# ChaissonLab/LRA

Measured on AMD Instinct MI355X. Metric: aligned Gbp/s, 30 kb ONT vs GRCh38 (MapRead_lowacc end to end incl. SAM text), per job, higher is better.
Workload: dtype int32

## Files before the change

### lra_amd/csrc/indel_refine.hip

```cpp
#include "common.h"
#include "scan.h"
#include <algorithm>
#include <stdlib.h>

int lra_aog_launch_device(lra_ctx* ctx, int n, const char* d_qseq, const char* d_tseq, const uint64_t* d_q_off,
                          const int32_t* d_q_len, const uint64_t* d_t_off, const int32_t* d_t_len, const int32_t* d_k,
                          int m, int mm, int indel, int32_t* d_score, int32_t* d_nblocks, int32_t* d_blocks,
                          const uint64_t* d_block_off, int32_t* d_status);

namespace {

constexpr int BAD = -999999999;
constexpr int NEG = -2000000000;
enum { C_DIAG = 0, C_LEFT = 1, C_DOWN = 2, C_BOUND = 3, C_DELCLOSE = 4, C_INSCLOSE = 5, C_DONE = 6 };

__device__ __forceinline__ void wave_sync() {
  __builtin_amdgcn_fence(__ATOMIC_RELEASE, "workgroup");
  __builtin_amdgcn_wave_barrier();
  __builtin_amdgcn_fence(__ATOMIC_ACQUIRE, "workgroup");
}

__device__ __forceinline__ void wave_sync_lds() {
  __builtin_amdgcn_fence(__ATOMIC_RELEASE, "wavefront");
  __builtin_amdgcn_wave_barrier();
// ... 307 lines not shown
  int status = B.s_status[s];
  const long tLen = (long)B.s_rows[s];
  Row* rows = B.rows + B.s_row_off[s];
  unsigned long long cells = 0;
  int width = 0;
  if (!status && tLen > 0) {
    int run = 0x7fffffff;
    for (long base = ((tLen - 1) / 64) * 64; base >= 0; base -= 64) {
      const long r = base + lane;
      const int own = (r < tLen) ? rows[r].S : 0x7fffffff;
      int v = own;
      for (int d = 1; d < 64; d <<= 1) { int o = __shfl_down(v, d); if (lane + d < 64) v = min(v, o); }
      v = min(v, run);
      if (r < tLen && v != own) rows[r].S = v;
      run = __shfl(v, 0);
    }
    const int a = B.s_aln[s];
    const unsigned char* tb = (const unsigned char*)B.tseq + B.t_off[a] + B.s_tStart[s];
    int runE = -0x7fffffff;
    for (long base = 0; base < tLen; base += 64) {
      const long r = base + lane;
      Row w; w.S = 0; w.E = -0x7fffffff; w.C = 0; w.T = 0;
      if (r < tLen) w = rows[r];
      int e = w.E;
      for (int d = 1; d < 64; d <<= 1) { int o = __shfl_up(e, d); if (lane >= d) e = max(e, o); }
      e = max(e, runE);
      runE = __shfl(e, 63);
      int len = (r < tLen) ? e - w.S + 1 : 0;
      if (r < tLen) {
        if (len < 1 || w.S < 0) status |= 1;
        else if (len > MAXW) status |= 4;
        width = max(width, len);
      }
      const unsigned long long l = (unsigned long long)max(len, 0);
      unsigned long long inc = l;
      for (int d = 1; d < 64; d <<= 1) { unsigned long long o = __shfl_up(inc, d); if (lane >= d) inc += o; }
      if (r < tLen) { w.E = e; w.C = (unsigned int)(cells + inc - l); w.T = tb[r]; rows[r] = w; }
      cells += __shfl(inc, 63);
    }
    for (int o = 32; o > 0; o >>= 1) { status |= __shfl_xor(status, o); width = max(width, __shfl_xor(width, o)); }
  }
  if (lane == 0) {
    B.s_cells[s] = status ? 0 : cells;
    B.s_status[s] = status;
    B.s_width[s] = status ? 0 : width;
    B.s_tmpcap[s] = status ? 0 : (uint64_t)(tLen + ((long)B.s_qEnd[s] - B.s_qStart[s]) + 2);
  }
}

constexpr int FILL_BINS = 128;
template <bool EMIT>
__global__ void ir_classify(uint64_t n_seg, const int32_t* __restrict__ s_kind, const int32_t* __restrict__ s_status, const int32_t* __restrict__ s_width,
                            const uint64_t* __restrict__ s_rows, int* bins, uint32_t* list) {
  const uint64_t s = (uint64_t)blockIdx.x * blockDim.x + threadIdx.x;
  const int lane = threadIdx.x & 63;
  int bin = -1;
  if (s < n_seg && s_kind[s] == 0 && s_status[s] == 0) {
    const int w = s_width[s];
    const uint32_t r = (uint32_t)min((unsigned long long)s_rows[s], 0x7fffffffULL);
    bin = (w <= 16 ? 0 : w <= 32 ? 1 : w <= 64 ? 2 : 3) * 32 + (r ? __clz(r) : 31);
  }
  const unsigned long long below = (lane == 0) ? 0ULL : (~0ULL >> (64 - lane));
  unsigned long long todo = __ballot(bin >= 0);
  while (todo) {
    const int leader = __ffsll((long long)todo) - 1;
    const int b = __shfl(bin, leader);
    const unsigned long long m = __ballot(bin == b);
    int base = 0;
    if (lane == leader) base = atomicAdd(&bins[b], __popcll(m));
    base = __shfl(base, leader);
    if (EMIT && bin == b) list[base + __popcll(m & below)] = (uint32_t)s;
    todo &= ~m;
  }
}

struct FillArgs {
  uint64_t n_seg;
  const int32_t* s_aln; const uint64_t* s_rows; const uint64_t* s_row_off; const uint64_t* s_cell_off;
  const Row* rows;
  const char* qseq; const uint64_t* q_off; const int32_t* q_len;
  int match, mismatch, g;
  unsigned char* path;
  const uint32_t* list; int* cursor;
};

__device__ __forceinline__ bool is_bound(long row, int c, int len) { return c == len - 1 || (row > 0 && c == 0); }

__device__ __forceinline__ int shr1(int x, int fill) { return __builtin_amdgcn_update_dpp(fill, x, 0x138, 0xf, 0xf, false); }
template <int G>
__device__ __forceinline__ int scan_max(int w) {
  w = max(w, __builtin_amdgcn_update_dpp(NEG, w, 0x111, 0xf, 0xf, false));
  w = max(w, __builtin_amdgcn_update_dpp(NEG, w, 0x112, 0xf, 0xf, false));
  w = max(w, __builtin_amdgcn_update_dpp(NEG, w, 0x114, 0xf, 0xf, false));
  w = max(w, __builtin_amdgcn_update_dpp(NEG, w, 0x118, 0xf, 0xf, false));
  if (G >= 32) w = max(w, __builtin_amdgcn_update_dpp(NEG, w, 0x142, 0xa, 0xf, false));
  if (G >= 64) w = max(w, __builtin_amdgcn_update_dpp(NEG, w, 0x143, 0xc, 0xf, false));
  return w;
}

template <int G>
__global__ void __launch_bounds__(64) ir_fill(FillArgs F) {
  constexpr int GP = 64 / G;
  constexpr int CLS = (G == 16) ? 0 : (G == 32) ? 1 : 2;
  const int lane = threadIdx.x;
  const int c = lane % G, gbase = lane - c;
  const int g = F.g, go = 2 * F.g + 1;
  const long listEnd = F.cursor[4 + CLS];
  const uint32_t* list = F.list;
  long ti = -1, tLen = 0;
  const Row* rows = nullptr; const unsigned char* qb = nullptr; unsigned char* P = nullptr;
  long chunkBase = 0, qLast = 0;
  Row chunk; chunk.S = chunk.E = chunk.T = 0; chunk.C = 0;
  int W0 = 0, qlo = 0, qhi = 0, qnext = 0;
  int prevM = BAD, prevD = BAD, prevS = 0, prevLen = 0;
  bool done = false;
  auto ldq = [&](long idx) -> int { return qb[idx < qLast ? idx : qLast]; };
  while (true) {
    if (!done && ti < 0) {
      long x = 0;
      if (c == 0) x = atomicAdd(&F.cursor[CLS], 1);
      x = __shfl(x, gbase);
      if (x < listEnd) {
        const uint64_t s = list[x];
        const int a = F.s_aln[s];
        tLen = (long)F.s_rows[s];
        rows = F.rows + F.s_row_off[s];
        qb = (const unsigned char*)F.qseq + F.q_off[a];
        qLast = (long)F.q_len[a] - 1;
        P = F.path + F.s_cell_off[s];
        ti = 0; chunkBase = 0;
        if (c < tLen) chunk = rows[c];
        W0 = rows[0].S;
        qlo = ldq((long)W0 + c); qhi = ldq((long)W0 + G + c); qnext = ldq((long)W0 + 2 * G + c);
      } else done = true;
    }
    if (__ballot(!done) == 0ULL) break;
    if (!done && ti - chunkBase == G) { chunkBase = ti; if (ti + c < tLen) chunk = rows[ti + c]; }
    const int src = gbase + (int)((ti - chunkBase) & (G - 1));
    const int S = __shfl(chunk.S, src), E = __shfl(chunk.E, src), tch = __shfl(chunk.T, src);
    const unsigned int C = __shfl(chunk.C, src);
    while (!done && S - W0 >= G) { W0 += G; qlo = qhi; qhi = qnext; qnext = ldq((long)W0 + 2 * G + c); }
    const int j = S - W0 + c;
    const int q1 = __shfl(qlo, gbase + (j & (G - 1))), q2 = __shfl(qhi, gbase + (j & (G - 1)));
    const int qch = (j < G) ? q1 : q2;
    const int len = E - S + 1;
    const bool lastRow = (ti == tLen - 1);
    const int off = S - prevS;
    const bool interior = c >= 1 && (lastRow ? c <= len - 1 : c <= len - 2);
    const int srcA = c + off, srcD = srcA - 1;
    const bool aboveIn = srcA <= prevLen - 1;
    const int aM = __shfl(prevM, gbase + (srcA & (G - 1))), aD = __shfl(prevD, gbase + (srcA & (G - 1)));
    const int dM = shr1(aM, BAD);
    const bool okA = aboveIn && !is_bound(ti - 1, srcA, prevLen);
    const bool okD = aboveIn && srcD >= 0 && !is_bound(ti - 1, srcD, prevLen);
    const int dOpen = okA ? aM + go : BAD, dExt = okA ? aD : BAD;
    const int Dv = max(dOpen, dExt);
    const int delOpen = (Dv == dOpen) ? 1 : 0;
    const int mS = okD ? dM + (tch == qch ? F.match : F.mismatch) : BAD;
    const int dS = okA ? aM + g : BAD;
    const int V = interior ? max(mS, max(dS, Dv)) : NEG;
    const int W = scan_max<G>(V);
    int Wm1 = shr1(W, NEG), Vm1 = shr1(V, NEG);
    if (c == 0) { Wm1 = NEG; Vm1 = NEG; }
    const int Iv = max(BAD, go + Wm1);
    int M = max(max(BAD, V), max(Vm1 + g, go + Wm1));
    if (!interior) M = BAD;
// ... 40 lines not shown
    const uint64_t s = F.list[x];
    const int a = F.s_aln[s];
    const long tLen = (long)F.s_rows[s];
    const Row* rows = F.rows + F.s_row_off[s];
    const unsigned char* qb = (const unsigned char*)F.qseq + F.q_off[a];
    const long qLast = (long)F.q_len[a] - 1;
    unsigned char* P = F.path + F.s_cell_off[s];
    int prevS = 0, prevLen = 0;
    for (long ti = 0; ti < tLen; ti++) {
      const Row rw = rows[ti];
      const int S = rw.S, len = rw.E - rw.S + 1, tch = rw.T;
      const unsigned int C = rw.C;
      const bool lastRow = (ti == tLen - 1);
      const int off = S - prevS;
      const int cur = (int)(ti & 1), prv = cur ^ 1;
      int carryW = NEG, carryV = NEG, carryM = BAD;
      for (int base = 0; base < len; base += 64) {
        const int c = base + lane;
        int outM, outD; unsigned char outB;
        if (ti == 0) {
          const bool last0 = (c == len - 1) && (tLen > 1);
          outM = last0 ? BAD : (c == 0 ? 0 : c * g);
          outD = BAD;
          outB = (unsigned char)(last0 ? C_BOUND : (c == 0 ? C_DONE : C_LEFT));
        } else {
          const long qi = (long)S + c;
          const int qch = qb[qi < qLast ? qi : qLast];
          const bool interior = c >= 1 && (lastRow ? c <= len - 1 : c <= len - 2);
          const int srcA = c + off, srcD = srcA - 1;
          const bool aboveIn = srcA <= prevLen - 1;
          const bool inA = srcA >= 0 && srcA < prevLen, inD = srcD >= 0 && srcD < prevLen;
          const int aM = inA ? sM[prv][srcA] : BAD, aD = inA ? sD[prv][srcA] : BAD;
          const int dM = inD ? sM[prv][srcD] : BAD;
          const bool okA = aboveIn && !is_bound(ti - 1, srcA, prevLen);
          const bool okD = aboveIn && srcD >= 0 && !is_bound(ti - 1, srcD, prevLen);
          const int dOpen = okA ? aM + go : BAD, dExt = okA ? aD : BAD;
          const int Dv = max(dOpen, dExt);
          const int delOpen = (Dv == dOpen) ? 1 : 0;
          const int mS = okD ? dM + (tch == qch ? F.match : F.mismatch) : BAD;
          const int dS = okA ? aM + g : BAD;
          const int V = interior ? max(mS, max(dS, Dv)) : NEG;
          const int W = max(scan_max<64>(V), carryW);
          int Wm1 = shr1(W, NEG), Vm1 = shr1(V, NEG);
          if (lane == 0) { Wm1 = carryW; Vm1 = carryV; }
          if (c == 0) { Wm1 = NEG; Vm1 = NEG; }
          const int Iv = max(BAD, go + Wm1);
          int M = max(max(BAD, V), max(Vm1 + g, go + Wm1));
          if (!interior) M = BAD;
          int Mleft = shr1(M, BAD);
          if (lane == 0) Mleft = carryM;
          if (c <= 1) Mleft = BAD;
          const int iOpen = Mleft + go;
          const int insOpen = (Iv == iOpen) ? 1 : 0;
          const int iS = Mleft + g;
          int code;
          if (!interior) code = C_BOUND;
          else if (M == mS) code = C_DIAG;
          else if (M == iS) code = C_LEFT;
          else if (M == dS) code = C_DOWN;
          else if (M == Dv) code = C_DELCLOSE;
          else code = C_INSCLOSE;
          outM = M; outD = interior ? Dv : BAD;
          outB = (unsigned char)(code | (delOpen << 3) | (insOpen << 4));
          carryW = __shfl(W, 63); carryV = __shfl(V, 63); carryM = __shfl(M, 63);
        }
        if (c < len) { P[C + c] = outB; sM[cur][c] = outM; sD[cur][c] = outD; }
      }
      wave_sync_lds();
      prevS = S; prevLen = len;
    }
  }
}

template <int N>
__device__ __forceinline__ int ror(int x) { return __builtin_amdgcn_update_dpp(0, x, 0x120 + N, 0xf, 0xf, true); }
__device__ __forceinline__ int pin(int x) { asm volatile("" : "+v"(x)); return x; }
__device__ __forceinline__ int ring_scan_max(int w, int d) {
  { const int t = pin(max(w, ror<1>(w))); w = (d >= 1) ? t : w; }
  { const int t = pin(max(w, ror<2>(w))); w = (d >= 2) ? t : w; }
  { const int t = pin(max(w, ror<4>(w))); w = (d >= 4) ? t : w; }
  { const int t = pin(max(w, ror<8>(w))); w = (d >= 8) ? t : w; }
  return w;
}
template <int NP>
__global__ void __launch_bounds__(64) ir_fill_cols(FillArgs F) {
  constexpr int G = 16;
  constexpr int CLS = NP - 1;
  const int lane = threadIdx.x;
  const int c = lane % G, gbase = lane - c;
  const int g = F.g, go = 2 * F.g + 1;
  const long listEnd = F.cursor[4 + CLS];
  const uint32_t* list = F.list;
  long ti = -1, tLen = 0;
  const Row* rows = nullptr; const unsigned char* qb = nullptr; unsigned char* P = nullptr;
  long qLast = 0;
  __shared__ Row s_chunk[64];
  long chunkBase = 0;
  Row chunk; chunk.S = chunk.E = chunk.T = 0; chunk.C = 0;
  int K0 = 0, q0 = 0, q1 = 0, q2 = 0, q3 = 0;
  int pM[NP], pD[NP], prevS = 0, prevLen = 0;
  for (int p = 0; p < NP; p++) { pM[p] = BAD; pD[p] = BAD; }
  bool done = false;
  auto ldq = [&](long idx) -> int { return qb[idx < qLast ? idx : qLast]; };
  while (true) {
    if (!done && ti < 0) {
      long x = 0;
      if (c == 0) x = atomicAdd(&F.cursor[CLS], 1);
      x = __shfl(x, gbase);
      if (x < listEnd) {
        const uint64_t s = list[x];
        const int a = F.s_aln[s];
        tLen = (long)F.s_rows[s];
        rows = F.rows + F.s_row_off[s];
        qb = (const unsigned char*)F.qseq + F.q_off[a];
        qLast = (long)F.q_len[a] - 1;
        P = F.path + F.s_cell_off[s];
        ti = 0; chunkBase = -G;
        if (c < tLen) chunk = rows[c];
        K0 = rows[0].S >> 4;
        const long b = 16L * K0 + c;
        q0 = ldq(b); q1 = ldq(b + G); q2 = ldq(b + 2 * G); q3 = ldq(b + 3 * G);
      } else done = true;
    }
    if (__ballot(!done) == 0ULL) break;
    if (!done && ti - chunkBase == G) {
      chunkBase = ti;
      s_chunk[lane] = chunk;
      wave_sync_lds();
      if (ti + G + c < tLen) chunk = rows[ti + G + c];
    }
    const Row rw = s_chunk[gbase + (int)((ti - chunkBase) & (G - 1))];
    const int S = rw.S, E = rw.E, tch = rw.T;
    const unsigned int C = rw.C;
    if (!done && (S >> 4) != K0) {
      const int adv = (S >> 4) - K0;
      K0 = S >> 4;
      const long b = 16L * K0 + c;
      if (adv == 1) { q0 = q1; q1 = q2; q2 = q3; }
      else { q0 = ldq(b); q1 = ldq(b + G); q2 = ldq(b + 2 * G); }
      q3 = ldq(b + 3 * G);
    }
    const int len = E - S + 1;
    const bool lastRow = (ti == tLen - 1);
    const int off = S - prevS;
    const int d = (c - S) & (G - 1);
    const bool head = (d == 0);
    const bool lo = c >= (S & (G - 1));
    int nM[NP], nD[NP];
    for (int p = 0; p < NP; p++) { nM[p] = BAD; nD[p] = BAD; }
    int cW = NEG, cV = NEG, cM = BAD, cA = BAD;
    for (int p = 0; p < NP; p++) {
      if (p == 1 && len <= G) break;
      const int cc = d + G * p;
      const int qch = (p == 0) ? (lo ? q0 : q1) : (lo ? q1 : q2);
      const bool interior = cc >= 1 && (lastRow ? cc <= len - 1 : cc <= len - 2);
      const int srcA = cc + off, srcD = srcA - 1;
      const bool aboveIn = srcA <= prevLen - 1;
      const int aM = (NP > 1 && srcA >= G) ? pM[NP - 1] : pM[0];
      const int aD = (NP > 1 && srcA >= G) ? pD[NP - 1] : pD[0];
      const int rA = pin(ror<1>(aM));
      const int dM = (p == 1 && head) ? cA : rA;
      const bool okA = aboveIn && !is_bound(ti - 1, srcA, prevLen);
      const bool okD = aboveIn && srcD >= 0 && !is_bound(ti - 1, srcD, prevLen);
      const int dOpen = okA ? aM + go : BAD, dExt = okA ? aD : BAD;
      const int Dv = max(dOpen, dExt);
      const int delOpen = (Dv == dOpen) ? 1 : 0;
      const int mS = okD ? dM + (tch == qch ? F.match : F.mismatch) : BAD;
      const int dS = okA ? aM + g : BAD;
      const int V = interior ? max(mS, max(dS, Dv)) : NEG;
      const int W = ring_scan_max((p == 1 && head) ? max(V, cW) : V, d);
      const int rW = pin(ror<1>(W)), rV = pin(ror<1>(V));
      const int Wm1 = head ? cW : rW, Vm1 = head ? cV : rV;
      const int Iv = max(BAD, go + Wm1);
      int M = max(max(BAD, V), max(Vm1 + g, go + Wm1));
      if (!interior) M = BAD;
      const int rM = pin(ror<1>(M));
      int Mleft = head ? cM : rM;
      if (cc <= 1) Mleft = BAD;
      const int iOpen = Mleft + go;
      const int insOpen = (Iv == iOpen) ? 1 : 0;
      const int iS = Mleft + g;
      int code;
      if (!interior) code = C_BOUND;
      else if (M == mS) code = C_DIAG;
      else if (M == iS) code = C_LEFT;
      else if (M == dS) code = C_DOWN;
      else if (M == Dv) code = C_DELCLOSE;
      else code = C_INSCLOSE;
      int outM = M, outD = interior ? Dv : BAD;
      unsigned char outB = (unsigned char)(code | (delOpen << 3) | (insOpen << 4));
      if (ti == 0) {
        const bool last0 = (cc == len - 1) && (tLen > 1);
        outM = last0 ? BAD : (cc == 0 ? 0 : cc * g);
        outD = BAD;
        outB = (unsigned char)(last0 ? C_BOUND : (cc == 0 ? C_DONE : C_LEFT));
      }
      if (!done && cc < len) P[C + cc] = outB;
      nM[p] = outM; nD[p] = outD;
      if (NP > 1 && p == 0) { cW = rW; cV = rV; cM = rM; cA = rA; }
    }
    if (!done) {
      for (int p = 0; p < NP; p++) { pM[p] = nM[p]; pD[p] = nD[p]; }
      prevS = S; prevLen = len;
      ti++;
      if (ti == tLen) ti = -1;
    }
  }
}

struct TraceArgs {
  uint64_t n_seg;
  const int32_t* s_kind; const int32_t* s_tStart; const uint64_t* s_rows; const uint64_t* s_row_off;
  const uint64_t* s_cells; const uint64_t* s_cell_off; int32_t* s_status;
  const Row* rows;
  const unsigned char* path;
  uint32_t* s_nblk;
  const uint64_t* s_tmp_off; int32_t* tmp_blocks;
};

constexpr int TW_ROWS = 128, TW_PATH = 4096;
__global__ void __launch_bounds__(64) ir_trace_wave(TraceArgs T) {
  __shared__ Row s_rows[TW_ROWS];
  __shared__ __attribute__((aligned(16))) unsigned char s_path[TW_PATH + 16];
  const int lane = threadIdx.x;
  const uint64_t s = blockIdx.x;
  if (s >= T.n_seg) return;
  if (T.s_kind[s] != 0) return;
  if (T.s_status[s] != 0) { if (lane == 0) T.s_nblk[s] = 0; return; }
  const long tLen = (long)T.s_rows[s];
  const Row* rows = T.rows + T.s_row_off[s];
  const unsigned char* P = T.path + T.s_cell_off[s];
  int32_t* ob = T.tmp_blocks + 3 * T.s_tmp_off[s];
  const long cap = (long)(T.s_tmp_off[s + 1] - T.s_tmp_off[s]);
  long ti = tLen - 1;
  long rBase = 0, wLo = 1, wHi = 0; unsigned pBase = 0;
  auto stage = [&](long at) {
    wave_sync();
    wHi = at; rBase = max(0L, at - TW_ROWS + 1);
    for (long x = lane; x <= at - rBase; x += 64) s_rows[x] = rows[rBase + x];
    wave_sync();
    const Row last = s_rows[at - rBase];
    const unsigned end = last.C + (unsigned)max(last.E - last.S + 1, 0);
    long lo = rBase, hi = at;
    while (lo < hi) { const long mid = (lo + hi) >> 1; if (end - s_rows[mid - rBase].C <= (unsigned)TW_PATH) hi = mid; else lo = mid + 1; }
    wLo = lo; pBase = s_rows[lo - rBase].C;
    const unsigned nbytes = min(end - pBase, (unsigned)TW_PATH);
    const unsigned char* start = P + pBase;
    const unsigned delta = (unsigned)((uintptr_t)start & 15);
    const uint4* a16 = (const uint4*)(start - delta);
    const unsigned full = (delta + nbytes) >> 4;
    for (unsigned x = lane; x < full; x += 64) ((uint4*)s_path)[x] = a16[x];
    for (unsigned x = (full << 4) + lane; x < delta + nbytes; x += 64) s_path[x] = (start - delta)[x];
    pBase -= delta;
    wave_sync();
  };
  stage(ti);
  Row rw = s_rows[ti - rBase];
  int qa = rw.E;
  int mat = 0;
  int bad = 0;
  long nblk = 0;
  long q = (long)rw.E + 1, t = (long)T.s_tStart[s] + tLen;
  int curKind = -1, pending = 0;
  long dlen = 0;
  long steps = 0;
  const long step_cap = 4 * (long)T.s_cells[s] + 64;
  auto emit_block = [&]() {
    if (nblk < cap) { if (lane == 0) { ob[3 * nblk] = (int)q; ob[3 * nblk + 1] = (int)t; ob[3 * nblk + 2] = (int)dlen; } } else bad = 1;
    nblk++;
  };
  auto op = [&](int kind, long times) {
    if (kind != curKind) {
      if (curKind == -1 && kind == 0) { pending = 1; dlen = 0; }
      if (kind != 0) {
        if (pending) emit_block();
        pending = 1; dlen = 0;
      }
      curKind = kind;
    }
    if (kind == 0) { dlen += times; q -= times; t -= times; }
    else if (kind == 1) q -= times;
    else t -= times;
  };
  while (true) {
    if (ti < wLo || ti > wHi) stage(ti);
    rw = s_rows[ti - rBase];
    if (mat == 0) {
      const long tl = ti - lane;
      bool fast = false;
// ... 141 lines not shown


struct Arena {
  char* base; size_t cap, used;
  template <typename T> T* get(size_t n) {
    size_t bytes = (n * sizeof(T) + 255) & ~(size_t)255;
    if (used + bytes > cap) return nullptr;
    T* p = (T*)(base + used);
    used += bytes;
    return p;
  }
};

}

template <typename CT>
static void scan(lra_ctx* ctx, long n, const CT* c, uint64_t* off) {
  (void)lra_exclusive_scan<CT>(ctx, n, c, off);
}

static int d2h(lra_ctx* ctx, void* dst, const void* src, size_t bytes) {
  LRA_HIP_CHECK(ctx, hipMemcpyAsync(dst, src, bytes, hipMemcpyDeviceToHost, ctx->stream));
  LRA_HIP_CHECK(ctx, hipStreamSynchronize(ctx->stream));
  return LRA_OK;
}

extern "C" int lra_indel_refine_batch(lra_ctx* ctx, int n_aln, const int32_t* d_blocks_in, const uint64_t* d_block_off, uint64_t n_blocks_in,
                                      const char* d_qseq, const uint64_t* d_q_off, const int32_t* d_q_len, const char* d_tseq,
                                      const uint64_t* d_t_off, const int64_t* d_t_len, int refine_band, int match, int mismatch,
                                      int indel, int end_align, lra_refine_result* out) {
  if (!ctx || !out || n_aln < 0) return LRA_ERR_INVALID;
  if (refine_band < 2 || refine_band > 64) return lra_set_err(ctx, LRA_ERR_INVALID, "refine_band must be 2..64");
  if (indel >= 0) return lra_set_err(ctx, LRA_ERR_INVALID, "indel score must be negative");
  memset(out, 0, sizeof(*out));
  if (n_aln == 0) return LRA_OK;
  LRA_HIP_CHECK(ctx, hipSetDevice(ctx->device));
  hipStream_t st = ctx->stream;
  const size_t nA = (size_t)n_aln, nBk = (size_t)n_blocks_in + 2 * nA;
  const size_t perAln = ((nA * 4 + 255) & ~(size_t)255) * 3 + (((nA + 1) * 8 + 255) & ~(size_t)255) * 3;
  char* baseP = (char*)lra_ensure(ctx, 70, perAln + 4096);
  if (!baseP) return LRA_ERR_NOMEM;
  Arena ap{baseP, perAln + 4096, 0};
  IRArgs A;
  memset(&A, 0, sizeof A);
  A.n_aln = n_aln; A.blocks_in = d_blocks_in; A.block_off = d_block_off;
  A.qseq = d_qseq; A.q_off = d_q_off; A.q_len = d_q_len; A.tseq = d_tseq; A.t_off = d_t_off; A.t_len = d_t_len;
  A.k = refine_band; A.match = match; A.mismatch = mismatch; A.indel = indel; A.endAlign = end_align;
  A.a_nseg = ap.get<uint32_t>(nA); A.a_nitem = ap.get<uint32_t>(nA); A.a_status = ap.get<int32_t>(nA);
  uint64_t* seg_off = ap.get<uint64_t>(nA + 1); uint64_t* item_off = ap.get<uint64_t>(nA + 1); uint64_t* out_block_off = ap.get<uint64_t>(nA + 1);
  if (!out_block_off) return lra_set_err(ctx, LRA_ERR_NOMEM, "arena accounting");
  A.seg_off = seg_off; A.item_off = item_off;
  const int nbA = (n_aln + SEG_LANES - 1) / SEG_LANES;
  lra_time_begin(ctx, "ir_segment");
  hipLaunchKernelGGL(ir_segment<false>, dim3(nbA), dim3(64), 0, st, A);
  lra_time_end(ctx);
  scan(ctx, (long)n_aln, A.a_nseg, seg_off);
  scan(ctx, (long)n_aln, A.a_nitem, item_off);
  uint64_t n_seg = 0, n_item = 0;
  if (d2h(ctx, &n_seg, seg_off + n_aln, 8) || d2h(ctx, &n_item, item_off + n_aln, 8)) return LRA_ERR_HIP;
  const size_t capSeg = (size_t)n_seg + 1, capItem = (size_t)n_item + 1;
  size_t needA = 0;
  auto add = [&](size_t n, size_t sz) { needA += ((n * sz + 255) & ~(size_t)255); };
  add(3 * nBk, 4);
  for (int i = 0; i < 8; i++) add(capSeg, 4);
  add(3 * capSeg, 4); add(capSeg, 4); add(capSeg, 8); add(capSeg, 4);
  add(capSeg + 1, 8); add(capSeg + 1, 8); add(capSeg, 8); add(capSeg + 1, 8); add(capSeg, 4);
  add(capSeg, 4); add(capSeg, 4); add(capSeg, 8); add(capSeg + 1, 8); add(capSeg, 4); add(capSeg + 1, 8);
  add(capSeg, 4); add(FILL_BINS + 8, 4);
  add(capItem, 4); add(3 * capItem, 4); add(capItem, 4); add(capItem, 4); add(capItem + 1, 8);
  add(capSeg, 8); add(capSeg, 4); add(capSeg, 8); add(capSeg, 4); add(capSeg, 4); add(capSeg, 4); add(capSeg + 1, 8);
  add(capSeg, 4); add(capSeg, 4); add(capSeg, 4);
  add(capSeg, 4); add(capSeg + 1, 8);
  char* baseA = (char*)lra_scratch(ctx, 2, needA + 4096);
  if (!baseA) return LRA_ERR_NOMEM;
  Arena ar{baseA, needA + 4096, 0};
  A.ab = ar.get<int32_t>(3 * nBk);
  A.s_aln = ar.get<int32_t>(capSeg); A.s_kind = ar.get<int32_t>(capSeg); A.s_qStart = ar.get<int32_t>(capSeg); A.s_tStart = ar.get<int32_t>(capSeg);
  A.s_qEnd = ar.get<int32_t>(capSeg); A.s_tEnd = ar.get<int32_t>(capSeg); A.s_b0 = ar.get<int32_t>(capSeg); A.s_b1 = ar.get<int32_t>(capSeg);
  A.s_first = ar.get<int32_t>(3 * capSeg); A.s_lastLen = ar.get<int32_t>(capSeg); A.s_rows = ar.get<uint64_t>(capSeg); A.s_isAog = ar.get<uint32_t>(capSeg);
  uint64_t* s_row_off = ar.get<uint64_t>(capSeg + 1); uint64_t* s_aog_off = ar.get<uint64_t>(capSeg + 1);
  uint64_t* s_cells = ar.get<uint64_t>(capSeg); uint64_t* s_cell_off = ar.get<uint64_t>(capSeg + 1); int32_t* s_status = ar.get<int32_t>(capSeg);
  uint32_t* s_nblk = ar.get<uint32_t>(capSeg); int32_t* s_width = ar.get<int32_t>(capSeg); uint64_t* s_tmpcap = ar.get<uint64_t>(capSeg);
  uint64_t* s_tmp_off = ar.get<uint64_t>(capSeg + 1); uint32_t* s_aog_idx = ar.get<uint32_t>(capSeg); uint64_t* s_out_off = ar.get<uint64_t>(capSeg + 1);
  uint32_t* fill_lists = ar.get<uint32_t>(capSeg); int* fill_counts = ar.get<int>(FILL_BINS + 8);
  A.i_kind = ar.get<int32_t>(capItem); A.i_data = ar.get<int32_t>(3 * capItem);
  int32_t* i_aln = ar.get<int32_t>(capItem); uint32_t* i_count = ar.get<uint32_t>(capItem); uint64_t* i_out_off = ar.get<uint64_t>(capItem + 1);
  uint64_t* p_q_off = ar.get<uint64_t>(capSeg); int32_t* p_q_len = ar.get<int32_t>(capSeg); uint64_t* p_t_off = ar.get<uint64_t>(capSeg);
  int32_t* p_t_len = ar.get<int32_t>(capSeg); int32_t* p_k = ar.get<int32_t>(capSeg); uint32_t* p_cap = ar.get<uint32_t>(capSeg);
  uint64_t* p_block_off = ar.get<uint64_t>(capSeg + 1);
  int32_t* p_score = ar.get<int32_t>(capSeg); int32_t* p_nblocks = ar.get<int32_t>(capSeg); int32_t* p_status = ar.get<int32_t>(capSeg);
  uint32_t* s_nchunk = ar.get<uint32_t>(capSeg); uint64_t* chunk_off = ar.get<uint64_t>(capSeg + 1);
  if (!chunk_off) return lra_set_err(ctx, LRA_ERR_NOMEM, "arena accounting");
  lra_time_begin(ctx, "ir_segment");
  hipLaunchKernelGGL(ir_segment<true>, dim3(nbA), dim3(64), 0, st, A);
  lra_time_end(ctx);
  hipLaunchKernelGGL(ir_item_aln, dim3((n_aln + 255) / 256), dim3(256), 0, st, n_aln, item_off, i_aln);
  uint64_t n_rows = 0, n_aog = 0, n_cells = 0;
  const int32_t* tmp_blocks = nullptr;
  if (n_seg) {
    scan(ctx, (long)n_seg, A.s_rows, s_row_off);
    scan(ctx, (long)n_seg, A.s_isAog, s_aog_off);
    if (d2h(ctx, &n_rows, s_row_off + n_seg, 8) || d2h(ctx, &n_aog, s_aog_off + n_seg, 8)) return LRA_ERR_HIP;
    Row* rows = (Row*)lra_ensure(ctx, 0, (n_rows + 1) * sizeof(Row));
    if (!rows) return LRA_ERR_NOMEM;
    BandArgs B;
    B.n_seg = n_seg; B.s_aln = A.s_aln; B.s_kind = A.s_kind; B.s_qStart = A.s_qStart; B.s_qEnd = A.s_qEnd; B.s_tStart = A.s_tStart;
    B.s_b0 = A.s_b0; B.s_b1 = A.s_b1; B.s_first = A.s_first; B.s_lastLen = A.s_lastLen; B.s_rows = A.s_rows; B.s_row_off = s_row_off;
    B.ab = A.ab; B.block_off = d_block_off; B.tseq = d_tseq; B.t_off = d_t_off; B.k = refine_band; B.rows = rows;
    B.s_cells = s_cells; B.s_status = s_status; B.s_width = s_width; B.s_tmpcap = s_tmpcap;
    const unsigned gridL = (unsigned)((n_seg + 63) / 64);
    const unsigned gridS = (unsigned)((n_seg + 255) / 256);
    lra_time_begin(ctx, "ir_band");
    B.s_nchunk = s_nchunk; B.chunk_off = chunk_off; B.n_task = 0; B.task_seg = nullptr; B.chunkT = nullptr; B.chunkQ = nullptr;
    hipLaunchKernelGGL(ir_band_nchunk, dim3(gridS), dim3(256), 0, st, B);
    scan(ctx, (long)n_seg, s_nchunk, chunk_off);
    uint64_t n_task = 0;
    if (d2h(ctx, &n_task, chunk_off + n_seg, 8)) return LRA_ERR_HIP;
    uint32_t* task_seg = (uint32_t*)lra_ensure(ctx, 54, (n_task + 1) * 4);
    int32_t* chunk_tq = (int32_t*)lra_ensure(ctx, 55, (n_task + 1) * 8);
    if (!task_seg || !chunk_tq) return LRA_ERR_NOMEM;
    B.n_task = n_task; B.task_seg = task_seg; B.chunkT = chunk_tq; B.chunkQ = chunk_tq + n_task + 1;
    hipLaunchKernelGGL(ir_band_tasks, dim3(gridS), dim3(256), 0, st, B);
    hipLaunchKernelGGL(ir_band_prep, dim3((unsigned)n_seg), dim3(64), 0, st, B);
    if (n_task) {
      const unsigned gridT = (unsigned)((n_task + 63) / 64);
      if (refine_band <= 8) hipLaunchKernelGGL(ir_band_chunk<16>, dim3(gridT), dim3(64), 0, st, B);
      else if (refine_band <= 32) hipLaunchKernelGGL(ir_band_chunk<64>, dim3(gridT), dim3(64), 0, st, B);
      else hipLaunchKernelGGL(ir_band_chunk<128>, dim3(gridT), dim3(64), 0, st, B);
    }
    hipLaunchKernelGGL(ir_band_scan, dim3((unsigned)n_seg), dim3(64), 0, st, B);
    lra_time_end(ctx);
    scan(ctx, (long)n_seg, s_cells, s_cell_off);
    scan(ctx, (long)n_seg, s_tmpcap, s_tmp_off);
    uint64_t n_tmp = 0;
    if (d2h(ctx, &n_cells, s_cell_off + n_seg, 8) || d2h(ctx, &n_tmp, s_tmp_off + n_seg, 8)) return LRA_ERR_HIP;
    const size_t pathBytes = (n_cells + 256 + 255) & ~(size_t)255;
    unsigned char* path = (unsigned char*)lra_ensure(ctx, 12, pathBytes + (n_tmp + 1) * 12 + 256);
    if (!path) return LRA_ERR_NOMEM;
    int32_t* tmpb = (int32_t*)(path + pathBytes);
    tmp_blocks = tmpb;
    int h_bins[FILL_BINS], h_start[FILL_BINS], h_cursor[8] = {0, 0, 0, 0, 0, 0, 0, 0};
    LRA_HIP_CHECK(ctx, hipMemsetAsync(fill_counts, 0, FILL_BINS * 4, st));
    hipLaunchKernelGGL(ir_classify<false>, dim3((unsigned)((n_seg + 255) / 256)), dim3(256), 0, st, n_seg, A.s_kind, s_status, s_width, A.s_rows, fill_counts, fill_lists);
    if (d2h(ctx, h_bins, fill_counts, FILL_BINS * 4)) return LRA_ERR_HIP;
    { int run = 0; for (int b = 0; b < FILL_BINS; b++) { h_start[b] = run; run += h_bins[b]; if ((b & 31) == 0) h_cursor[b / 32] = h_start[b]; if ((b & 31) == 31) h_cursor[4 + b / 32] = run; } }
    LRA_HIP_CHECK(ctx, hipMemcpyAsync(fill_counts, h_start, FILL_BINS * 4, hipMemcpyHostToDevice, st));
    hipLaunchKernelGGL(ir_classify<true>, dim3((unsigned)((n_seg + 255) / 256)), dim3(256), 0, st, n_seg, A.s_kind, s_status, s_width, A.s_rows, fill_counts, fill_lists);
    int* fill_cursor = fill_counts + FILL_BINS;
    LRA_HIP_CHECK(ctx, hipMemcpyAsync(fill_cursor, h_cursor, 32, hipMemcpyHostToDevice, st));
    FillArgs F;
    F.n_seg = n_seg; F.s_aln = A.s_aln; F.s_rows = A.s_rows; F.s_row_off = s_row_off; F.s_cell_off = s_cell_off; F.rows = rows;
    F.qseq = d_qseq; F.q_off = d_q_off; F.q_len = d_q_len; F.match = match; F.mismatch = mismatch; F.g = indel; F.path = path;
    F.list = fill_lists; F.cursor = fill_cursor;
    const unsigned cap_grid = (unsigned)ctx->num_cu * 32;
    if (getenv("LRA_IR_DBG")) {
      const int hc[4] = {h_cursor[4] - h_cursor[0], h_cursor[5] - h_cursor[1], h_cursor[6] - h_cursor[2], h_cursor[7] - h_cursor[3]};
      fprintf(stderr, "[ir] n_seg %llu n_rows %llu n_cells %llu n_task %llu n_item %llu fill classes 16/32/64/wide: %d %d %d %d\n",
              (unsigned long long)n_seg, (unsigned long long)n_rows, (unsigned long long)n_cells, (unsigned long long)n_task,
              (unsigned long long)n_item, hc[0], hc[1], hc[2], hc[3]);
    }
    lra_time_begin(ctx, "ir_fill");
    const uint64_t n16 = (uint64_t)(h_cursor[4] - h_cursor[0]), n32 = (uint64_t)(h_cursor[5] - h_cursor[1]), n64 = (uint64_t)(h_cursor[6] - h_cursor[2]);
    const uint64_t nWide = (uint64_t)(h_cursor[7] - h_cursor[3]);
    if (n16) hipLaunchKernelGGL(ir_fill_cols<1>, dim3((unsigned)std::min<uint64_t>((n16 + 3) / 4, cap_grid)), dim3(64), 0, lra_side_fork(ctx, 1), F);
    if (n64) hipLaunchKernelGGL(ir_fill<64>, dim3((unsigned)std::min<uint64_t>(n64, cap_grid)), dim3(64), 0, lra_side_fork(ctx, 2), F);
    if (nWide) hipLaunchKernelGGL(ir_fill_wide, dim3((unsigned)std::min<uint64_t>(nWide, cap_grid)), dim3(64), 0, lra_side_fork(ctx, 3), F);
    if (n32) hipLaunchKernelGGL(ir_fill_cols<2>, dim3((unsigned)std::min<uint64_t>((n32 + 3) / 4, cap_grid)), dim3(64), 0, st, F);
    if (n16) lra_side_join(ctx, 1);
    if (n64) lra_side_join(ctx, 2);
    if (nWide) lra_side_join(ctx, 3);
    lra_time_end(ctx);
    TraceArgs T;
    T.n_seg = n_seg; T.s_kind = A.s_kind; T.s_tStart = A.s_tStart; T.s_rows = A.s_rows; T.s_row_off = s_row_off;
    T.s_cells = s_cells; T.s_cell_off = s_cell_off; T.s_status = s_status; T.rows = rows; T.path = path;
    T.s_nblk = s_nblk; T.s_tmp_off = s_tmp_off; T.tmp_blocks = tmpb;
    lra_time_begin(ctx, "ir_trace");
    hipLaunchKernelGGL(ir_trace_wave, dim3((unsigned)n_seg), dim3(64), 0, st, T);
    lra_time_end(ctx);
    if (n_aog) {
      hipLaunchKernelGGL(ir_aog_setup, dim3((unsigned)((n_seg + 255) / 256)), dim3(256), 0, st, n_seg, A.s_kind, A.s_aln, s_aog_off, A.s_qStart,
                         A.s_tStart, A.s_qEnd, A.s_tEnd, d_q_off, d_t_off, refine_band, s_aog_idx, p_q_off, p_q_len, p_t_off, p_t_len, p_k, p_cap);
      scan(ctx, (long)n_aog, p_cap, p_block_off);
      uint64_t aog_cap = 0;
      if (d2h(ctx, &aog_cap, p_block_off + n_aog, 8)) return LRA_ERR_HIP;
      if (aog_cap * 12 + 64 > ctx->aux_bytes) {
        if (ctx->aux) (void)hipFree(ctx->aux);
        ctx->aux = nullptr; ctx->aux_bytes = 0;
        size_t want = aog_cap * 12 + aog_cap * 3 + 4096;
        if (hipMalloc(&ctx->aux, want) != hipSuccess) return lra_set_err(ctx, LRA_ERR_NOMEM, "aog block buffer");
        ctx->aux_bytes = want;
      }
      int rc = lra_aog_launch_device(ctx, (int)n_aog, d_qseq, d_tseq, p_q_off, p_q_len, p_t_off, p_t_len, p_k, match, mismatch, indel, p_score,
                                     p_nblocks, (int32_t*)ctx->aux, p_block_off, p_status);
      if (rc) return rc;
    }
  }
  hipLaunchKernelGGL(ir_item_counts, dim3((unsigned)((n_item + 255) / 256)), dim3(256), 0, st, n_item, A.i_kind, A.i_data, i_aln, seg_off, A.s_kind,
                     s_nblk, s_aog_idx, p_nblocks, i_count);
  scan(ctx, (long)n_item, i_count, i_out_off);
  uint64_t n_out = 0;
  if (d2h(ctx, &n_out, i_out_off + n_item, 8)) return LRA_ERR_HIP;
  if ((n_out + 1) * 12 > ctx->out_bytes) {
    if (ctx->out_buf) (void)hipFree(ctx->out_buf);
    ctx->out_buf = nullptr; ctx->out_bytes = 0;
    size_t want = (n_out + 1) * 12 + (n_out + 1) * 3 + 4096;
    if (hipMalloc(&ctx->out_buf, want) != hipSuccess) return lra_set_err(ctx, LRA_ERR_NOMEM, "refined block buffer");
    ctx->out_bytes = want;
  }
  int32_t* out_blocks = (int32_t*)ctx->out_buf;
  hipLaunchKernelGGL(ir_finalize_offsets, dim3((unsigned)((std::max<uint64_t>(n_item, nA + 1) + 255) / 256)), dim3(256), 0, st, n_aln, n_item, item_off,
                     i_out_off, A.i_kind, A.i_data, i_aln, seg_off, s_out_off, out_block_off);
  GatherArgs G;
  G.n_item = n_item; G.i_kind = A.i_kind; G.i_data = A.i_data; G.i_aln = i_aln; G.i_out_off = i_out_off; G.seg_off = seg_off;
  G.s_kind = A.s_kind; G.s_qStart = A.s_qStart; G.s_tStart = A.s_tStart; G.s_aog_idx = s_aog_idx;
  G.aog_blocks = (const int32_t*)ctx->aux; G.aog_block_off = p_block_off; G.aog_nblocks = p_nblocks;
  G.tmp_blocks = tmp_blocks; G.s_tmp_off = s_tmp_off; G.s_nblk = s_nblk; G.out_blocks = out_blocks;
  lra_time_begin(ctx, "ir_gather");
  if (n_item) hipLaunchKernelGGL(ir_gather, dim3((unsigned)std::min<uint64_t>(n_item, 65535 * 4)), dim3(64), 0, st, G);
  lra_time_end(ctx);
  hipLaunchKernelGGL(ir_aln_status, dim3((n_aln + 255) / 256), dim3(256), 0, st, n_aln, seg_off, A.s_kind, s_status, s_aog_idx, p_status, A.a_status);
  LRA_HIP_CHECK(ctx, hipGetLastError());
  LRA_HIP_CHECK(ctx, hipStreamSynchronize(st));
  out->n_aln = n_aln; out->n_blocks = n_out; out->n_segments = n_seg; out->n_cells = n_cells; out->n_rows = n_rows; out->n_aog = n_aog;
  out->d_block_off = out_block_off; out->d_blocks = out_blocks; out->d_status = A.a_status;
  return LRA_OK;
}
```

Measured before the change: 1.091.

## Add lean single-pass row loop to narrow column fill kernel

When a 16-row chunk is loaded, the kernel classifies each row as ordinary (interior, band width at most 16, query window advancing by 0 or 1 block). While every active group's current row is ordinary, a tight inner loop runs a single-pass DP row with no NP loop, no first-row special case and a cheap query-register slide. The kernel also narrows index arithmetic from 64-bit to 32-bit and marks segments with overflowed row counts as failed instead of filling them. Optional per-kernel iteration counters are compiled in only behind a debug environment variable.

```diff
diff --git a/lra_amd/csrc/indel_refine.hip b/lra_amd/csrc/indel_refine.hip
--- a/lra_amd/csrc/indel_refine.hip
+++ b/lra_amd/csrc/indel_refine.hip
@@ -413,6 +413,8 @@
   int match, mismatch, g;
   unsigned char* path;
   const uint32_t* list; int* cursor;
+  int32_t* s_status;
+  unsigned long long* dbg;
 };
 
 __device__ __forceinline__ bool is_bound(long row, int c, int len) { return c == len - 1 || (row > 0 && c == 0); }
@@ -619,60 +621,130 @@
   { const int t = pin(max(w, ror<8>(w))); w = (d >= 8) ? t : w; }
   return w;
 }
-template <int NP>
+template <int NP, bool COUNT>
 __global__ void __launch_bounds__(64) ir_fill_cols(FillArgs F) {
   constexpr int G = 16;
   constexpr int CLS = NP - 1;
   const int lane = threadIdx.x;
   const int c = lane % G, gbase = lane - c;
   const int g = F.g, go = 2 * F.g + 1;
-  const long listEnd = F.cursor[4 + CLS];
+  const int listEnd = F.cursor[4 + CLS];
   const uint32_t* list = F.list;
-  long ti = -1, tLen = 0;
+  int ti = -1, tLen = 0;
   const Row* rows = nullptr; const unsigned char* qb = nullptr; unsigned char* P = nullptr;
-  long qLast = 0;
+  unsigned int qLast = 0;
   __shared__ Row s_chunk[64];
-  long chunkBase = 0;
+  int chunkBase = 0;
   Row chunk; chunk.S = chunk.E = chunk.T = 0; chunk.C = 0;
+  unsigned int ordMask = 0, slideMask = 0;
   int K0 = 0, q0 = 0, q1 = 0, q2 = 0, q3 = 0;
   int pM[NP], pD[NP], prevS = 0, prevLen = 0;
   for (int p = 0; p < NP; p++) { pM[p] = BAD; pD[p] = BAD; }
   bool done = false;
-  auto ldq = [&](long idx) -> int { return qb[idx < qLast ? idx : qLast]; };
+  unsigned long long nLean = 0, nGeneral = 0, nRefill = 0, nFetch = 0;
+  auto ldq = [&](unsigned int idx) -> int { return qb[idx < qLast ? idx : qLast]; };
   while (true) {
-    if (!done && ti < 0) {
-      long x = 0;
+    bool fetched = false;
+    while (!done && ti < 0) {
+      int x = 0;
       if (c == 0) x = atomicAdd(&F.cursor[CLS], 1);
       x = __shfl(x, gbase);
       if (x < listEnd) {
         const uint64_t s = list[x];
-        const int a = F.s_aln[s];
-        tLen = (long)F.s_rows[s];
-        rows = F.rows + F.s_row_off[s];
-        qb = (const unsigned char*)F.qseq + F.q_off[a];
-        qLast = (long)F.q_len[a] - 1;
-        P = F.path + F.s_cell_off[s];
-        ti = 0; chunkBase = -G;
-        if (c < tLen) chunk = rows[c];
-        K0 = rows[0].S >> 4;
-        const long b = 16L * K0 + c;
-        q0 = ldq(b); q1 = ldq(b + G); q2 = ldq(b + 2 * G); q3 = ldq(b + 3 * G);
-      } else done = true;
+        if (F.s_rows[s] >> 31) {
+          if (c == 0) F.s_status[s] = 4;
+        } else {
+          const int a = F.s_aln[s];
+          tLen = (int)F.s_rows[s];
+          rows = F.rows + F.s_row_off[s];
+          qb = (const unsigned char*)F.qseq + F.q_off[a];
+          qLast = (unsigned int)(F.q_len[a] - 1);
+          P = F.path + F.s_cell_off[s];
+          ti = 0; chunkBase = -G;
+          if (c < tLen) chunk = rows[c];
+          K0 = rows[0].S >> 4;
+          const unsigned int b = 16u * (unsigned int)K0 + c;
+          q0 = ldq(b); q1 = ldq(b + G); q2 = ldq(b + 2 * G); q3 = ldq(b + 3 * G);
+          fetched = true;
+        }
+      } else { done = true; slideMask = 0; }
     }
     if (__ballot(!done) == 0ULL) break;
-    if (!done && ti - chunkBase == G) {
+    const bool refill = !done && ti - chunkBase == G;
+    if (refill) {
       chunkBase = ti;
       s_chunk[lane] = chunk;
       wave_sync_lds();
+      const int myLen = chunk.E - chunk.S + 1;
+      const int upLen = pin(ror<1>(myLen)), upS = pin(ror<1>(chunk.S));
+      const int aboveLen = c ? upLen : prevLen, aboveS = c ? upS : prevS;
+      const int r = ti + c, adv = (chunk.S >> 4) - (aboveS >> 4);
+      const bool ord = r >= 2 && r <= tLen - 2 && myLen <= G && aboveLen <= G && (adv == 0 || adv == 1);
+      ordMask = (unsigned int)(__ballot(ord) >> gbase) & 0xffffu;
+      slideMask = (unsigned int)(__ballot(ord && adv == 1) >> gbase) & 0xffffu;
       if (ti + G + c < tLen) chunk = rows[ti + G + c];
     }
-    const Row rw = s_chunk[gbase + (int)((ti - chunkBase) & (G - 1))];
+    int r = (ti - chunkBase) & (G - 1);
+    if (COUNT) {
+      if (__ballot(refill) != 0ULL) nRefill++;
+      if (__ballot(fetched) != 0ULL) nFetch++;
+    }
+    if (__ballot(!done && !((ordMask >> r) & 1u)) == 0ULL) {
+      do {
+        if (COUNT) nLean++;
+        const Row rw = s_chunk[gbase + r];
+        const int S = rw.S, E = rw.E, tch = rw.T;
+        const unsigned int C = rw.C;
+        if ((slideMask >> r) & 1u) {
+          asm volatile("v_mov_b32 %0, %1\n\tv_mov_b32 %1, %2\n\tv_mov_b32 %2, %3" : "+v"(q0), "+v"(q1), "+v"(q2) : "v"(q3));
+          K0++;
+          q3 = ldq(16u * (unsigned int)K0 + c + 3 * G);
+        }
+        const int len = E - S + 1;
+        const int off = S - prevS;
+        const int cc = (c - S) & (G - 1);
+        const bool head = (cc == 0);
+        const int qch = (c >= (S & (G - 1))) ? q0 : q1;
+        const bool interior = cc >= 1 && cc <= len - 2;
+        const int srcA = cc + off;
+        const int aM = pM[0], aD = pD[0];
+        const int dM = pin(ror<1>(aM));
+        const bool okA = srcA >= 1 && srcA <= prevLen - 2;
+        const bool okD = srcA >= 2 && srcA <= prevLen - 1;
+        const int dOpen = okA ? aM + go : BAD, dExt = okA ? aD : BAD;
+        const int Dv = max(dOpen, dExt);
+        const int delOpen = (Dv == dOpen) ? 1 : 0;
+        const int mS = okD ? dM + (tch == qch ? F.match : F.mismatch) : BAD;
+        const int dS = okA ? aM + g : BAD;
+        const int V = interior ? max(mS, max(dS, Dv)) : NEG;
+        const int W = ring_scan_max(V, cc);
+        const int rW = pin(ror<1>(W)), rV = pin(ror<1>(V));
+        const int Wm1 = head ? NEG : rW, Vm1 = head ? NEG : rV;
+        const int Iv = max(BAD, go + Wm1);
+        int M = max(max(BAD, V), max(Vm1 + g, go + Wm1));
+        if (!interior) M = BAD;
+        const int rM = pin(ror<1>(M));
+        const int Mleft = (cc <= 1) ? BAD : rM;
+        const int iOpen = Mleft + go;
+        const int insOpen = (Iv == iOpen) ? 1 : 0;
+        const int iS = Mleft + g;
+        int code = (M == mS) ? C_DIAG : (M == iS) ? C_LEFT : (M == dS) ? C_DOWN : (M == Dv) ? C_DELCLOSE : C_INSCLOSE;
+        if (!interior) code = C_BOUND;
+        if (!done && cc < len) P[C + cc] = (unsigned char)(code | (delOpen << 3) | (insOpen << 4));
+        pM[0] = M; pD[0] = interior ? Dv : BAD;
+        prevS = S; prevLen = len;
+        if (!done) { ti++; r++; }
+      } while (__builtin_amdgcn_ballot_w64(!done && !((ordMask >> r) & 1u)) == 0ULL);
+      continue;
+    }
+    if (COUNT) nGeneral++;
+    const Row rw = s_chunk[gbase + r];
     const int S = rw.S, E = rw.E, tch = rw.T;
     const unsigned int C = rw.C;
     if (!done && (S >> 4) != K0) {
       const int adv = (S >> 4) - K0;
       K0 = S >> 4;
-      const long b = 16L * K0 + c;
+      const unsigned int b = 16u * (unsigned int)K0 + c;
       if (adv == 1) { q0 = q1; q1 = q2; q2 = q3; }
       else { q0 = ldq(b); q1 = ldq(b + G); q2 = ldq(b + 2 * G); }
       q3 = ldq(b + 3 * G);
@@ -742,6 +814,10 @@
       ti++;
       if (ti == tLen) ti = -1;
     }
+  }
+  if (COUNT && lane == 0) {
+    atomicAdd(&F.dbg[4 * CLS + 0], nLean); atomicAdd(&F.dbg[4 * CLS + 1], nGeneral);
+    atomicAdd(&F.dbg[4 * CLS + 2], nRefill); atomicAdd(&F.dbg[4 * CLS + 3], nFetch);
   }
 }
 
@@ -1049,7 +1125,7 @@
   uint64_t* s_cells = ar.get<uint64_t>(capSeg); uint64_t* s_cell_off = ar.get<uint64_t>(capSeg + 1); int32_t* s_status = ar.get<int32_t>(capSeg);
   uint32_t* s_nblk = ar.get<uint32_t>(capSeg); int32_t* s_width = ar.get<int32_t>(capSeg); uint64_t* s_tmpcap = ar.get<uint64_t>(capSeg);
   uint64_t* s_tmp_off = ar.get<uint64_t>(capSeg + 1); uint32_t* s_aog_idx = ar.get<uint32_t>(capSeg); uint64_t* s_out_off = ar.get<uint64_t>(capSeg + 1);
-  uint32_t* fill_lists = ar.get<uint32_t>(capSeg); int* fill_counts = ar.get<int>(FILL_BINS + 8);
+  uint32_t* fill_lists = ar.get<uint32_t>(capSeg); int* fill_counts = ar.get<int>(FILL_BINS + 8 + 16);
   A.i_kind = ar.get<int32_t>(capItem); A.i_data = ar.get<int32_t>(3 * capItem);
   int32_t* i_aln = ar.get<int32_t>(capItem); uint32_t* i_count = ar.get<uint32_t>(capItem); uint64_t* i_out_off = ar.get<uint64_t>(capItem + 1);
   uint64_t* p_q_off = ar.get<uint64_t>(capSeg); int32_t* p_q_len = ar.get<int32_t>(capSeg); uint64_t* p_t_off = ar.get<uint64_t>(capSeg);
@@ -1118,9 +1194,14 @@
     FillArgs F;
     F.n_seg = n_seg; F.s_aln = A.s_aln; F.s_rows = A.s_rows; F.s_row_off = s_row_off; F.s_cell_off = s_cell_off; F.rows = rows;
     F.qseq = d_qseq; F.q_off = d_q_off; F.q_len = d_q_len; F.match = match; F.mismatch = mismatch; F.g = indel; F.path = path;
-    F.list = fill_lists; F.cursor = fill_cursor;
+    F.list = fill_lists; F.cursor = fill_cursor; F.s_status = s_status;
+    F.dbg = (unsigned long long*)(fill_counts + FILL_BINS + 8);
+    const bool fill_dbg = getenv("LRA_IR_DBG") != nullptr;
+    void (*const fill_cols1)(FillArgs) = fill_dbg ? ir_fill_cols<1, true> : ir_fill_cols<1, false>;
+    void (*const fill_cols2)(FillArgs) = fill_dbg ? ir_fill_cols<2, true> : ir_fill_cols<2, false>;
     const unsigned cap_grid = (unsigned)ctx->num_cu * 32;
-    if (getenv("LRA_IR_DBG")) {
+    if (fill_dbg) {
+      LRA_HIP_CHECK(ctx, hipMemsetAsync(F.dbg, 0, 64, st));
       const int hc[4] = {h_cursor[4] - h_cursor[0], h_cursor[5] - h_cursor[1], h_cursor[6] - h_cursor[2], h_cursor[7] - h_cursor[3]};
       fprintf(stderr, "[ir] n_seg %llu n_rows %llu n_cells %llu n_task %llu n_item %llu fill classes 16/32/64/wide: %d %d %d %d\n",
               (unsigned long long)n_seg, (unsigned long long)n_rows, (unsigned long long)n_cells, (unsigned long long)n_task,
@@ -1129,14 +1210,20 @@
     lra_time_begin(ctx, "ir_fill");
     const uint64_t n16 = (uint64_t)(h_cursor[4] - h_cursor[0]), n32 = (uint64_t)(h_cursor[5] - h_cursor[1]), n64 = (uint64_t)(h_cursor[6] - h_cursor[2]);
     const uint64_t nWide = (uint64_t)(h_cursor[7] - h_cursor[3]);
-    if (n16) hipLaunchKernelGGL(ir_fill_cols<1>, dim3((unsigned)std::min<uint64_t>((n16 + 3) / 4, cap_grid)), dim3(64), 0, lra_side_fork(ctx, 1), F);
+    if (n16) hipLaunchKernelGGL(fill_cols1, dim3((unsigned)std::min<uint64_t>((n16 + 3) / 4, cap_grid)), dim3(64), 0, lra_side_fork(ctx, 1), F);
     if (n64) hipLaunchKernelGGL(ir_fill<64>, dim3((unsigned)std::min<uint64_t>(n64, cap_grid)), dim3(64), 0, lra_side_fork(ctx, 2), F);
     if (nWide) hipLaunchKernelGGL(ir_fill_wide, dim3((unsigned)std::min<uint64_t>(nWide, cap_grid)), dim3(64), 0, lra_side_fork(ctx, 3), F);
-    if (n32) hipLaunchKernelGGL(ir_fill_cols<2>, dim3((unsigned)std::min<uint64_t>((n32 + 3) / 4, cap_grid)), dim3(64), 0, st, F);
+    if (n32) hipLaunchKernelGGL(fill_cols2, dim3((unsigned)std::min<uint64_t>((n32 + 3) / 4, cap_grid)), dim3(64), 0, st, F);
     if (n16) lra_side_join(ctx, 1);
     if (n64) lra_side_join(ctx, 2);
     if (nWide) lra_side_join(ctx, 3);
     lra_time_end(ctx);
+    if (fill_dbg) {
+      unsigned long long h_dbg[8];
+      if (d2h(ctx, h_dbg, F.dbg, 64)) return LRA_ERR_HIP;
+      for (int np = 1; np <= 2; np++)
+        fprintf(stderr, "[ir] fill_cols<%d> iterations: lean %llu general %llu refill %llu fetch %llu\n", np, h_dbg[4 * np - 4], h_dbg[4 * np - 3], h_dbg[4 * np - 2], h_dbg[4 * np - 1]);
+    }
     TraceArgs T;
     T.n_seg = n_seg; T.s_kind = A.s_kind; T.s_tStart = A.s_tStart; T.s_rows = A.s_rows; T.s_row_off = s_row_off;
     T.s_cells = s_cells; T.s_cell_off = s_cell_off; T.s_status = s_status; T.rows = rows; T.path = path;
```

After: 1.099 (median of 6 runs). No clear change (+0.7%).
